# struan-robertson/shoeprint-image-retrieval

Hardware: AMD Instinct MI355X
Metric: query x gallery NCC pairs/sec (higher is better)
Workload: dtype f32; 1 GPU; config 2: WVU2019-shaped VGG16 conv3_3 NCC: Q=100 x G=1500 (1500/GPU), features [256,128,64] stored as float32, rotations/scales none, queries signal 1 / noise 126; method=fft, gallery_chunk=1500, storage=float32, parallelism=gallery-shard x1, streams=1

## Files before the change

### shoeprint-image-retrieval_amd/csrc/ncc_prep6.hip

```cpp
#include "fft_core.h"
#include "ncc_fft_cfg.h"
#include "ncc_prep_common.h"

namespace spr {
namespace {

using C6 = Cfg<12, 16, 12, 8, 384, 5, 2, 1>;
constexpr int kPT = 512;
constexpr int kLoads = 16;
constexpr int kSeg = 4;
constexpr int kRowSeg = 16;
constexpr int kChansPerWg = 8;

#ifdef SPR_PREP6_STAMPS
__device__ unsigned long long g_prep6_stamps[16];
#define SPR_PSTAMP6(i) do { if (blockIdx.x == 12 && blockIdx.y == 700 && c == c_first + 1 && threadIdx.x == 0) g_prep6_stamps[i] = __builtin_amdgcn_s_memtime(); } while (0)
#else
#define SPR_PSTAMP6(i)
#endif

struct Prep6Lds {
  size_t x0_off, f_off, xbuf_off, tw_off, total;
  int f_stride;
};
Prep6Lds prep6_lds(const NccGeom& g) {
  const int h = g.ih, w = g.iw;
  Prep6Lds l;
  l.f_stride = C6::NW / 2 + 1;
  const size_t f_bytes = sizeof(cf) * static_cast<size_t>(2 * ((h + 1) / 2)) * l.f_stride;
  l.x0_off = 64;
  l.f_off = align_up(l.x0_off + sizeof(float) * h * w, 16);
  l.xbuf_off = align_up(l.f_off + f_bytes, 16);
  const size_t fft_total = l.xbuf_off + sizeof(cf) * C6::prep_xbuf_elems(kPT);
  const size_t stat_total = l.f_off + 2 * sizeof(double) * static_cast<size_t>(h) * w;
  l.tw_off = align_up(fft_total > stat_total ? fft_total : stat_total, 16);
  l.total = l.tw_off + sizeof(cf) * (C6::NW + C6::NH);
  return l;
}

__device__ __forceinline__ void stretch_offsets(double t, int sg, int d, double& off, double& tot) {
  const double a = shfl_xor(t, d), b = shfl_xor(t, 2 * d), c = shfl_xor(t, 3 * d);
  off = 0.0;
  tot = 0.0;
#pragma unroll
  for (int j = 0; j < kSeg; ++j) {
    const double v = j == sg ? t : (j == (sg ^ 1) ? a : (j == (sg ^ 2) ? b : c));
    off += j < sg ? v : 0.0;
    tot += v;
  }
}

__global__ void __launch_bounds__(kPT)
prep6_gallery_kernel(NccGeom g, const void* __restrict__ maps, unsigned char* __restrict__ prepared, size_t item_bytes,
                     const cf* __restrict__ tw_h, const cf* __restrict__ tw_w, unsigned x0_off, unsigned f_off,
                     unsigned xbuf_off, unsigned tw_off, int f_stride) {
  using C = C6;
  using GH = typename C::GH;
  using GW = typename C::GW;
  unsigned char* lds = dyn_lds();
  double* red = reinterpret_cast<double*>(lds);
  float* x0 = reinterpret_cast<float*>(lds + x0_off);
  cf* F = reinterpret_cast<cf*>(lds + f_off);
  cf* xbuf = reinterpret_cast<cf*>(lds + xbuf_off);
  const int tid = static_cast<int>(threadIdx.x);
  const size_t item = blockIdx.y;
  const int h = g.ih, w = g.iw, n = h * w;
  double* H1 = reinterpret_cast<double*>(lds + f_off);
  double* H2 = H1 + n;
  const int c_first = static_cast<int>(blockIdx.x) * kChansPerWg;
  const int c_end = c_first + kChansPerWg < g.channels ? c_first + kChansPerWg : g.channels;

  unsigned char* item_base = prepared + item * item_bytes;
  const size_t spec_bytes = sizeof(cf) * static_cast<size_t>(g.channels) * C::kSpecPerChan;
  unsigned char* flags = item_base + spec_bytes + sizeof(float) * static_cast<size_t>(g.channels) * g.inv_per_chan;

  const int dy = kPT / w, dx = kPT - dy * w;
  const int y_first = tid / w, x_first = tid - y_first * w;
  float v[kLoads];
  auto request = [&](int c) {
    const size_t chan_base = (item * g.channels + c) * static_cast<size_t>(g.g_h) * g.g_w;
    int yy = y_first, xx = x_first;
#pragma unroll
    for (int k = 0; k < kLoads; ++k) {
      v[k] = tid + k * kPT < n
                 ? load_feature(maps, chan_base + static_cast<size_t>(yy + g.crop) * g.g_w + (xx + g.crop), g.dtype)
                 : 0.0f;
      xx += dx; yy += dy;
      if (xx >= w) { xx -= w; ++yy; }
    }
  };
  request(c_first);

  cf* twt_w = reinterpret_cast<cf*>(lds + tw_off);
  cf* twt_h = twt_w + C::NW;
  for (int k = tid; k < C::NW; k += kPT) twt_w[k] = tw_w[(k / C::TGW) * (k % C::TGW)];
  for (int k = tid; k < C::NH; k += kPT) twt_h[k] = tw_h[(k / C::TGH) * (k % C::TGH)];

  const int cy = g.th / 2, cx = g.tw / 2;
  const int above = g.th - cy, left = g.tw - cx;
  const double inv_n = 1.0 / (static_cast<double>(g.th) * static_cast<double>(g.tw));

  for (int c = c_first; c < c_end; ++c) {
    SPR_PSTAMP6(0);
    double s = 0.0;
#pragma unroll
    for (int k = 0; k < kLoads; ++k)
      if (tid + k * kPT < n) s += static_cast<double>(v[k]);
    const double total = block_sum(s, red);
    const float mean = static_cast<float>(total / static_cast<double>(n));
    double e = 0.0;
#pragma unroll
    for (int k = 0; k < kLoads; ++k) {
      if (tid + k * kPT < n) {
        const float d = v[k] - mean;
        x0[tid + k * kPT] = d;
        const float sq = d * d;
        e += static_cast<double>(sq);
      }
    }
    SPR_PSTAMP6(1);
    const float energy = static_cast<float>(block_sum(e, red));
    const float rs = energy > 0.0f ? static_cast<float>(1.0 / sqrt(static_cast<double>(energy))) : 0.0f;
    if (tid == 0) flags[c] = rs == 0.0f ? 1 : 0;
    if (c + 1 < c_end) request(c + 1);
    SPR_PSTAMP6(2);

    {
      const int tidv = opaque(tid);
      const int u = tidv < h * kSeg ? tidv : h * kSeg - 1;
      const bool live = tidv < h * kSeg;
      const int y = u / kSeg, sg = u - y * kSeg;
      const int wseg = (w + kSeg - 1) / kSeg;
      const int xa = sg * wseg < w ? sg * wseg : w;
      const int cnt = w - xa < wseg ? w - xa : wseg;
      const float* src = x0 + y * w;
      float tv[kRowSeg];
#pragma unroll
      for (int k = 0; k < kRowSeg; ++k) {
        const float t = src[xa + k < w ? xa + k : w - 1];
        tv[k] = k < cnt ? t : 0.0f;
      }
      double r1 = 0.0, r2 = 0.0;
#pragma unroll
      for (int k = 0; k < kRowSeg; ++k) {
        const float sq = tv[k] * tv[k];
        r1 += static_cast<double>(tv[k]);
        r2 += static_cast<double>(sq);
      }
      double q1, q2, t1, t2;
      stretch_offsets(r1, sg, 1, q1, t1);
      stretch_offsets(r2, sg, 1, q2, t2);
      double* h1 = H1 + y * w;
      double* h2 = H2 + y * w;
      if (live) {
#pragma unroll
        for (int k = 0; k < kRowSeg; ++k) {
          const float sq = tv[k] * tv[k];
          q1 += static_cast<double>(tv[k]);
          q2 += static_cast<double>(sq);
          const int kk = xa + k + 1;
          if (k < cnt && kk < w) {
            const int xl = kk - left;
            if (xl >= 0 && xl <= cx) { h1[xl] = q1; h2[xl] = q2; }
            const int xr = kk + cx;
            if (xr < w) { h1[xr] = t1 - q1; h2[xr] = t2 - q2; }
          }
        }
        if (cnt > 0 && xa + cnt == w) {
          int xl = w - left < 0 ? 0 : w - left;
          const int xe = cx < w - 1 ? cx : w - 1;
          for (; xl <= xe; ++xl) { h1[xl] = q1; h2[xl] = q2; }
        }
      }
    }
    __syncthreads();
    SPR_PSTAMP6(7);

    {
      const int tidv = opaque(tid);
      const int xcol = ((tidv >> 6) & 3) * 16 + (tidv & 15), csg = (tidv >> 4) & 3;
      const int hseg = (h + kSeg - 1) / kSeg;
      const int ya = csg * hseg < h ? csg * hseg : h;
      const int ycnt = xcol < w ? (h - ya < hseg ? h - ya : hseg) : 0;
      double* col = ((tidv >> 8) ? H2 : H1) + ya * w + (xcol < w ? xcol : w - 1);
      constexpr int B = 8;
      double r = 0.0;
      for (int k0 = 0; k0 < ycnt; k0 += B) {
        double t[B];
#pragma unroll
        for (int k = 0; k < B; ++k) t[k] = col[(k0 + k < ycnt ? k0 + k : ycnt - 1) * w];
#pragma unroll
        for (int k = 0; k < B; ++k) r += k0 + k < ycnt ? t[k] : 0.0;
      }
      double run, tot;
      stretch_offsets(r, csg, 16, run, tot);
      for (int k0 = 0; k0 < ycnt; k0 += B) {
        double t[B];
#pragma unroll
        for (int k = 0; k < B; ++k) t[k] = col[(k0 + k < ycnt ? k0 + k : ycnt - 1) * w];
#pragma unroll
        for (int k = 0; k < B; ++k) {
          run += k0 + k < ycnt ? t[k] : 0.0;
          col[(k0 + k < ycnt ? k0 + k : ycnt - 1) * w] = run;
        }
      }
    }
    __syncthreads();
    SPR_PSTAMP6(8);
    {
      float4* inv4 = reinterpret_cast<float4*>(item_base + spec_bytes) + static_cast<size_t>(c) * (g.inv_per_chan / 4);
      for (int idx4 = opaque(tid); idx4 < C::kInv6PerChan / 4; idx4 += kPT) {
        const int pp = idx4 / C::NT, lane6 = idx4 - pp * C::NT;
        const int l64 = lane6 & 63, rg = l64 / 3, tq = l64 - 3 * rg;
        const int row = (lane6 >> 6) * C::kRowGroups + rg, n1 = 3 * pp + tq;
        float o[4] = {0.0f, 0.0f, 0.0f, 0.0f};
        if (l64 < 63 && n1 < 16 && row < h) {
          const int b = (33 * n1) % 48;
          const int ma = tq == 1 ? b - 32 : b, mb = ma == n1 ? n1 + 16 : n1;
          const bool upper = row <= cy;
          const int hi = upper ? (row + above < h ? row + above : h) - 1 : h - 1;
          const int lo = upper ? 0 : row - cy - 1;
          const double* p1a = H1 + hi * w;
          const double* p1b = H1 + lo * w;
          const double* p2a = H2 + hi * w;
          const double* p2b = H2 + lo * w;
          double a1[4], b1[4], a2[4], b2[4];
#pragma unroll
          for (int e = 0; e < 4; ++e) {
            const int x = 2 * (e < 2 ? ma : mb) + (e & 1), xs = x < w ? x : w - 1;
            a1[e] = p1a[xs]; b1[e] = p1b[xs]; a2[e] = p2a[xs]; b2[e] = p2b[xs];
          }
#pragma unroll
          for (int e = 0; e < 4; ++e) {
            const int x = 2 * (e < 2 ? ma : mb) + (e & 1);
            const float r = inv_sigma_from_sums(upper ? a1[e] : a1[e] - b1[e], upper ? a2[e] : a2[e] - b2[e], inv_n);
            o[e] = x < w ? r : 0.0f;
          }
        }
        inv4[idx4] = float4{o[0], o[1], o[2], o[3]};
      }
    }
    __syncthreads();
    SPR_PSTAMP6(3);

    {
      const int tidv = opaque(tid);
      const int giw = tidv / C::TGW, t = tidv - giw * C::TGW;
      const LdsTwiddles<C::TGW> twr{twt_w, t};
      cf* gbuf = xbuf + giw * C::kRowGroupElems;
      cf* zb = gbuf;
      const int pairs = (h + 1) / 2;
      constexpr int kPairsPerRound = kPT / C::TGW;
      const int rounds = ceil_div(pairs, kPairsPerRound);
      for (int rr = 0; rr < rounds; ++rr) {
        const int pr = rr * kPairsPerRound + giw;
        const int ra = 2 * pr, rb = ra + 1;
        cf x[C::EW], y[GW::SPL][C::TGW];
#pragma unroll
        for (int m = 0; m < C::EW; ++m) {
          const int n2 = GW::in_index(t, m);
          const bool in = n2 < w;
          x[m].x = (in && ra < h) ? x0[ra * w + n2] : 0.0f;
          x[m].y = (in && rb < h) ? x0[rb * w + n2] : 0.0f;
        }
        group_fft<C::EW, C::TGW, -1>(x, y, t, twr, gbuf);
        wave_sync();
#pragma unroll
        for (int pp = 0; pp < GW::SPL; ++pp)
#pragma unroll
          for (int sidx = 0; sidx < C::TGW; ++sidx)
            if (GW::out_valid(t, pp)) zb[GW::out_index(t, pp, sidx)] = y[pp][sidx];
        wave_sync();
        if (pr < pairs) {
          for (int k = t; k <= C::NW / 2; k += C::TGW) {
            const cf zk = zb[k];
            const cf zm = zb[k == 0 ? 0 : C::NW - k];
            F[ra * f_stride + k] = cmake(0.5f * (zk.x + zm.x), 0.5f * (zk.y - zm.y));
            F[rb * f_stride + k] = cmake(0.5f * (zk.y + zm.y), 0.5f * (zm.x - zk.x));
          }
        }
        wave_sync();
      }
    }
    __syncthreads();
    SPR_PSTAMP6(4);

    {
      cf* spec = reinterpret_cast<cf*>(item_base) + static_cast<size_t>(c) * C::kSpecPerChan;
      const int tidv = opaque(tid);
      const int gi = tidv / C::TGH, t = tidv - gi * C::TGH;
      const LdsTwiddles<C::TGH> twc{twt_h, t};
      cf* gbuf = xbuf + gi * GH::kGroupElems;
      const int rows_f = 2 * ((h + 1) / 2);
      constexpr int kColsPerRound = kPT / C::TGH;
      constexpr int kRounds = (C::COLS + 1 + kColsPerRound - 1) / kColsPerRound;
      for (int rc = 0; rc < kRounds; ++rc) {
        const int j = rc * kColsPerRound + gi;
        const bool nyq = j == C::COLS;
        const bool active = j <= C::COLS;
        cf x[C::EH], y[GH::SPL][C::TGH];
#pragma unroll
        for (int m = 0; m < C::EH; ++m) {
          const int n1 = GH::in_index(t, m);
          x[m] = (active && n1 < rows_f) ? F[n1 * f_stride + j] : cmake(0.0f, 0.0f);
        }
        group_fft<C::EH, C::TGH, -1>(x, y, t, twc, gbuf);
        if (active) {
#pragma unroll
          for (int pp = 0; pp < GH::SPL; ++pp) {
            if (!GH::out_valid(t, pp)) continue;
#pragma unroll
            for (int sidx = 0; sidx < C::TGH; ++sidx) {
              const int k1 = GH::out_index(t, pp, sidx);
              spec[nyq ? C::kNyqOffset + k1 : C::spec_index(C::slot(j), k1)] = y[pp][sidx];
            }
          }
        }
      }
    }
    __syncthreads();
    SPR_PSTAMP6(5);
  }
}

}

bool prep6_covers(const NccGeom& g) {
  if (!g.six || g.big || !g.prep6) return false;
  if (g.nh != C6::NH || g.nw != C6::NW || g.nt != C6::NT) return false;
  if (g.th < g.ih || g.tw < g.iw) return false;
  if (g.ih > C6::kRows6 || g.ih * kSeg > kPT || g.iw > 64) return false;
  if (g.ih * g.iw > kLoads * kPT) return false;
  if (g.inv_per_chan != C6::kInv6PerChan) return false;
  return prep6_lds(g).total <= static_cast<size_t>(kLdsLimit);
}

int launch_prep6(const NccGeom& g, const PlanScratch& s, const PrepCall& c) {
  const Prep6Lds l = prep6_lds(g);
  const size_t item_bytes = prepared_gallery_item_bytes(g, SPR_NCC_FFT);
  (void)hipFuncSetAttribute(reinterpret_cast<const void*>(prep6_gallery_kernel),
                            hipFuncAttributeMaxDynamicSharedMemorySize, kLdsLimit);
  const size_t elem = g.dtype == SPR_F32 ? 4 : 2;
  const size_t raw_item_bytes = static_cast<size_t>(g.channels) * g.g_h * g.g_w * elem;
  const int64_t batch = 65535;
  for (int64_t first = 0; first < c.n; first += batch) {
    const int64_t m = c.n - first < batch ? c.n - first : batch;
    hipLaunchKernelGGL(prep6_gallery_kernel, dim3(ceil_div(g.channels, kChansPerWg), static_cast<unsigned>(m)), dim3(kPT),
                       l.total, c.stream, g,
                       static_cast<const void*>(static_cast<const unsigned char*>(c.maps) + first * raw_item_bytes),
                       static_cast<unsigned char*>(c.prepared) + first * item_bytes, item_bytes, s.tw_h, s.tw_w,
                       static_cast<unsigned>(l.x0_off), static_cast<unsigned>(l.f_off), static_cast<unsigned>(l.xbuf_off),
                       static_cast<unsigned>(l.tw_off), l.f_stride);
    const int rc = check_launch("prep6_gallery_kernel");
    if (rc != SPR_OK) return rc;
  }
  return SPR_OK;
}

#ifdef SPR_PREP6_STAMPS
extern "C" int spr_debug_read_prep_stamps(unsigned long long* host, int n) {
  return hipMemcpyFromSymbol(host, HIP_SYMBOL(g_prep6_stamps), sizeof(unsigned long long) * n) == hipSuccess ? 0 : -1;
}
#endif

}
```

Measured before the change: 275,200 pairs/s.

## Streamline prep6 box-sum passes with register-resident columns and hoisted load offsets

Precomputes the per-thread feature load offsets once instead of recomputing them per channel. It restructures the row-prefix scatter into branch-light code with a fast path for full-width templates. It makes the column prefix-sum load each column segment into registers once rather than reading LDS twice. It also makes the inverse-sigma pass handle two output quads per thread with shared row pointers and skips the unused lower-row loads in the upper region. The goal is less address arithmetic and fewer LDS accesses in the preprocessing kernel, at the cost of more registers and subtler boundary logic.

After: 277,600 pairs/s, median of 6. No clear change (+0.9%).

```diff
diff --git a/shoeprint-image-retrieval_amd/csrc/ncc_prep6.hip b/shoeprint-image-retrieval_amd/csrc/ncc_prep6.hip
--- a/shoeprint-image-retrieval_amd/csrc/ncc_prep6.hip
+++ b/shoeprint-image-retrieval_amd/csrc/ncc_prep6.hip
@@ -1,3 +1,5 @@
+#include <type_traits>
+
 #include "fft_core.h"
 #include "ncc_fft_cfg.h"
 #include "ncc_prep_common.h"
@@ -10,6 +12,8 @@
 constexpr int kLoads = 16;
 constexpr int kSeg = 4;
 constexpr int kRowSeg = 16;
+constexpr int kColSeg = 32;
+static_assert((C6::kRows6 + kSeg - 1) / kSeg <= kColSeg, "a column stretch must fit the registers");
 constexpr int kChansPerWg = 8;
 
 #ifdef SPR_PREP6_STAMPS
@@ -76,18 +80,24 @@
 
   const int dy = kPT / w, dx = kPT - dy * w;
   const int y_first = tid / w, x_first = tid - y_first * w;
+  unsigned off[kLoads];
+  {
+    int yy = y_first, xx = x_first;
+#pragma unroll
+    for (int k = 0; k < kLoads; ++k) {
+      off[k] = static_cast<unsigned>((yy + g.crop) * g.g_w + (xx + g.crop));
+      xx += dx; yy += dy;
+      if (xx >= w) { xx -= w; ++yy; }
+    }
+  }
   float v[kLoads];
   auto request = [&](int c) {
     const size_t chan_base = (item * g.channels + c) * static_cast<size_t>(g.g_h) * g.g_w;
-    int yy = y_first, xx = x_first;
-#pragma unroll
-    for (int k = 0; k < kLoads; ++k) {
+#pragma unroll
+    for (int k = 0; k < kLoads; ++k)
       v[k] = tid + k * kPT < n
-                 ? load_feature(maps, chan_base + static_cast<size_t>(yy + g.crop) * g.g_w + (xx + g.crop), g.dtype)
+                 ? load_feature(maps, chan_base + static_cast<unsigned>(opaque(static_cast<int>(off[k]))), g.dtype)
                  : 0.0f;
-      xx += dx; yy += dy;
-      if (xx >= w) { xx -= w; ++yy; }
-    }
   };
   request(c_first);
 
@@ -99,6 +109,8 @@
   const int cy = g.th / 2, cx = g.tw / 2;
   const int above = g.th - cy, left = g.tw - cx;
   const double inv_n = 1.0 / (static_cast<double>(g.th) * static_cast<double>(g.tw));
+
+  const bool plain_rows = g.tw == w && w > (kSeg - 1) * ((w + kSeg - 1) / kSeg);
 
   for (int c = c_first; c < c_end; ++c) {
     SPR_PSTAMP6(0);
@@ -133,43 +145,51 @@
       const int wseg = (w + kSeg - 1) / kSeg;
       const int xa = sg * wseg < w ? sg * wseg : w;
       const int cnt = w - xa < wseg ? w - xa : wseg;
-      const float* src = x0 + y * w;
-      float tv[kRowSeg];
+      const float* src = x0 + y * w + xa;
+      double d1[kRowSeg], d2[kRowSeg];
 #pragma unroll
       for (int k = 0; k < kRowSeg; ++k) {
-        const float t = src[xa + k < w ? xa + k : w - 1];
-        tv[k] = k < cnt ? t : 0.0f;
+        const float t = src[k];
+        const float tv = k < cnt ? t : 0.0f;
+        const float sq = tv * tv;
+        d1[k] = static_cast<double>(tv);
+        d2[k] = static_cast<double>(sq);
       }
       double r1 = 0.0, r2 = 0.0;
 #pragma unroll
       for (int k = 0; k < kRowSeg; ++k) {
-        const float sq = tv[k] * tv[k];
-        r1 += static_cast<double>(tv[k]);
-        r2 += static_cast<double>(sq);
+        r1 += d1[k];
+        r2 += d2[k];
       }
       double q1, q2, t1, t2;
       stretch_offsets(r1, sg, 1, q1, t1);
       stretch_offsets(r2, sg, 1, q2, t2);
       double* h1 = H1 + y * w;
-      double* h2 = H2 + y * w;
-      if (live) {
+      const int end = xa + cnt;
+      auto scatter = [&](auto plain) {
 #pragma unroll
         for (int k = 0; k < kRowSeg; ++k) {
-          const float sq = tv[k] * tv[k];
-          q1 += static_cast<double>(tv[k]);
-          q2 += static_cast<double>(sq);
-          const int kk = xa + k + 1;
-          if (k < cnt && kk < w) {
-            const int xl = kk - left;
-            if (xl >= 0 && xl <= cx) { h1[xl] = q1; h2[xl] = q2; }
-            const int xr = kk + cx;
-            if (xr < w) { h1[xr] = t1 - q1; h2[xr] = t2 - q2; }
-          }
-        }
-        if (cnt > 0 && xa + cnt == w) {
-          int xl = w - left < 0 ? 0 : w - left;
+          q1 += d1[k];
+          q2 += d2[k];
+          const int kk = xa + k + 1 < end ? xa + k + 1 : end;
+          const bool pre = kk >= left;
+          const int xo = kk + (pre ? -left : cx);
+          const double o1 = pre ? q1 : t1 - q1, o2 = pre ? q2 : t2 - q2;
+          if (decltype(plain)::value || (cnt > 0 && (pre || kk < w - cx))) {
+            h1[xo] = o1;
+            h1[xo + n] = o2;
+          }
+        }
+      };
+      if (!live) {
+      } else if (plain_rows) {
+        scatter(std::true_type{});
+      } else {
+        scatter(std::false_type{});
+        if (cnt > 0 && end == w) {
+          int xl = w - left + 1 < 0 ? 0 : w - left + 1;
           const int xe = cx < w - 1 ? cx : w - 1;
-          for (; xl <= xe; ++xl) { h1[xl] = q1; h2[xl] = q2; }
+          for (; xl <= xe; ++xl) { h1[xl] = q1; h1[xl + n] = q2; }
         }
       }
     }
@@ -183,25 +203,46 @@
       const int ya = csg * hseg < h ? csg * hseg : h;
       const int ycnt = xcol < w ? (h - ya < hseg ? h - ya : hseg) : 0;
       double* col = ((tidv >> 8) ? H2 : H1) + ya * w + (xcol < w ? xcol : w - 1);
+      const int last = ycnt > 0 ? ycnt - 1 : 0;
       constexpr int B = 8;
+      double t[kColSeg];
+      int at = 0;
+#pragma unroll
+      for (int k0 = 0; k0 < kColSeg; k0 += B) {
+        if (k0 < hseg) {
+#pragma unroll
+          for (int k = k0; k < k0 + B; ++k) {
+            t[k] = col[at];
+            at += k < last ? w : 0;
+          }
+        }
+      }
+      sched_fence();
       double r = 0.0;
-      for (int k0 = 0; k0 < ycnt; k0 += B) {
-        double t[B];
-#pragma unroll
-        for (int k = 0; k < B; ++k) t[k] = col[(k0 + k < ycnt ? k0 + k : ycnt - 1) * w];
-#pragma unroll
-        for (int k = 0; k < B; ++k) r += k0 + k < ycnt ? t[k] : 0.0;
+#pragma unroll
+      for (int k0 = 0; k0 < kColSeg; k0 += B) {
+        if (k0 < hseg) {
+#pragma unroll
+          for (int k = k0; k < k0 + B; ++k) {
+            t[k] = k < ycnt ? t[k] : 0.0;
+            r += t[k];
+          }
+        }
       }
       double run, tot;
       stretch_offsets(r, csg, 16, run, tot);
-      for (int k0 = 0; k0 < ycnt; k0 += B) {
-        double t[B];
-#pragma unroll
-        for (int k = 0; k < B; ++k) t[k] = col[(k0 + k < ycnt ? k0 + k : ycnt - 1) * w];
-#pragma unroll
-        for (int k = 0; k < B; ++k) {
-          run += k0 + k < ycnt ? t[k] : 0.0;
-          col[(k0 + k < ycnt ? k0 + k : ycnt - 1) * w] = run;
+      if (ycnt > 0) {
+        at = 0;
+#pragma unroll
+        for (int k0 = 0; k0 < kColSeg; k0 += B) {
+          if (k0 < hseg) {
+#pragma unroll
+            for (int k = k0; k < k0 + B; ++k) {
+              run += t[k];
+              col[at] = run;
+              at += k < last ? w : 0;
+            }
+          }
         }
       }
     }
@@ -209,35 +250,52 @@
     SPR_PSTAMP6(8);
     {
       float4* inv4 = reinterpret_cast<float4*>(item_base + spec_bytes) + static_cast<size_t>(c) * (g.inv_per_chan / 4);
-      for (int idx4 = opaque(tid); idx4 < C::kInv6PerChan / 4; idx4 += kPT) {
-        const int pp = idx4 / C::NT, lane6 = idx4 - pp * C::NT;
+      for (int u = opaque(tid); u < 3 * C::NT; u += kPT) {
+        const int pq = u / C::NT, lane6 = u - pq * C::NT;
         const int l64 = lane6 & 63, rg = l64 / 3, tq = l64 - 3 * rg;
-        const int row = (lane6 >> 6) * C::kRowGroups + rg, n1 = 3 * pp + tq;
-        float o[4] = {0.0f, 0.0f, 0.0f, 0.0f};
-        if (l64 < 63 && n1 < 16 && row < h) {
-          const int b = (33 * n1) % 48;
-          const int ma = tq == 1 ? b - 32 : b, mb = ma == n1 ? n1 + 16 : n1;
-          const bool upper = row <= cy;
-          const int hi = upper ? (row + above < h ? row + above : h) - 1 : h - 1;
-          const int lo = upper ? 0 : row - cy - 1;
-          const double* p1a = H1 + hi * w;
-          const double* p1b = H1 + lo * w;
-          const double* p2a = H2 + hi * w;
-          const double* p2b = H2 + lo * w;
-          double a1[4], b1[4], a2[4], b2[4];
-#pragma unroll
-          for (int e = 0; e < 4; ++e) {
-            const int x = 2 * (e < 2 ? ma : mb) + (e & 1), xs = x < w ? x : w - 1;
-            a1[e] = p1a[xs]; b1[e] = p1b[xs]; a2[e] = p2a[xs]; b2[e] = p2b[xs];
-          }
-#pragma unroll
-          for (int e = 0; e < 4; ++e) {
-            const int x = 2 * (e < 2 ? ma : mb) + (e & 1);
-            const float r = inv_sigma_from_sums(upper ? a1[e] : a1[e] - b1[e], upper ? a2[e] : a2[e] - b2[e], inv_n);
-            o[e] = x < w ? r : 0.0f;
-          }
-        }
-        inv4[idx4] = float4{o[0], o[1], o[2], o[3]};
+        const int row = (lane6 >> 6) * C::kRowGroups + rg;
+        const bool in = l64 < 63 && row < h;
+        const bool upper = row <= cy;
+        const int hi = upper ? (row + above < h ? row + above : h) - 1 : h - 1;
+        const int lo = upper ? 0 : row - cy - 1;
+        const double* pa = H1 + hi * w;
+        const double* pb = H1 + lo * w;
+#pragma unroll
+        for (int half = 0; half < 2; ++half) {
+          const int pp = 2 * pq + half, n1 = 3 * pp + tq;
+          float o[4] = {0.0f, 0.0f, 0.0f, 0.0f};
+          if (in && n1 < 16) {
+            const int b = (33 * n1) % 48;
+            const int ma = tq == 1 ? b - 32 : b, mb = ma == n1 ? n1 + 16 : n1;
+            int x[4], xs[4];
+#pragma unroll
+            for (int e = 0; e < 4; ++e) {
+              x[e] = 2 * (e < 2 ? ma : mb) + (e & 1);
+              xs[e] = x[e] < w ? x[e] : w - 1;
+            }
+            double s1[4], s2[4];
+            if (upper) {
+#pragma unroll
+              for (int e = 0; e < 4; ++e) {
+                s1[e] = pa[xs[e]]; s2[e] = pa[xs[e] + n];
+              }
+            } else {
+              double b1[4], b2[4];
+#pragma unroll
+              for (int e = 0; e < 4; ++e) {
+                s1[e] = pa[xs[e]]; b1[e] = pb[xs[e]]; s2[e] = pa[xs[e] + n]; b2[e] = pb[xs[e] + n];
+              }
+#pragma unroll
+              for (int e = 0; e < 4; ++e) { s1[e] -= b1[e]; s2[e] -= b2[e]; }
+            }
+#pragma unroll
+            for (int e = 0; e < 4; ++e) {
+              const float r = inv_sigma_from_sums(s1[e], s2[e], inv_n);
+              o[e] = x[e] < w ? r : 0.0f;
+            }
+          }
+          inv4[pp * C::NT + lane6] = float4{o[0], o[1], o[2], o[3]};
+        }
       }
     }
     __syncthreads();
```
